# hjsuh94/irs_mpc

Hardware: NVIDIA B200
Metric: smoothed_dynamics_samples_per_s (higher is better)
Workload: dtype f32

## Files before the change

include/irs_mpc_b200.h:

```cpp
#ifndef IRS_MPC_B200_H
#define IRS_MPC_B200_H

#ifdef __cplusplus
extern "C" {
#endif

#define IRS_ABI_VERSION 3

enum { IRS_PENDULUM = 0, IRS_BICYCLE = 1, IRS_QUADROTOR = 2, IRS_THREE_CART = 3, IRS_MLP_2_1 = 4 };

int irs_mlp_register(int dim_x, int dim_u, int h1, int h2, const float* W1, const float* b1, const float* W2,
                     const float* b2, const float* W3, const float* b3, int* handle);
int irs_mlp_release(int handle);

enum {
  IRS_SAMPLES_BATCH_VARIANT = 1,
  IRS_PROJECT_ABSOLUTE = 2,
  IRS_PROJECT_DELTA = 4,
  IRS_ANTITHETIC = 8,
  IRS_CENTERED = 16
};

int irs_abi_version(void);
const char* irs_last_error(void);

int irs_set_gram_engine(int engine);

int irs_system_dims(int system, int* n, int* m, int* nj);

int irs_partial_width(int system, int order);

int irs_smooth_plan(int system, int order, int P, long long N, long long chunk_samples, int* C, long long* S);

int irs_smooth_zero_order_accumulate(int system, const double* params_host, int nparams, int flags,
                                     const double* x_nom, const double* u_nom, int P, long long N,
                                     const float* sigma_host, const float* noise,
                                     unsigned long long seed, unsigned iter, unsigned stream_id,
                                     unsigned p0, unsigned long long i0,
                                     int C, long long S, float* partials, void* stream);

int irs_smooth_first_order_accumulate(int system, const double* params_host, int nparams, int flags,
                                      const double* x_nom, const double* u_nom, int P, long long N,
                                      const float* sigma_host, const float* noise,
                                      unsigned long long seed, unsigned iter, unsigned stream_id,
                                      unsigned p0, unsigned long long i0,
                                      int C, long long S, float* partials, void* stream);

int irs_smooth_reduce_chunks(int system, int order, const float* partials, int P, int C,
                             double* reduced, void* stream);

int irs_smooth_finalize(int system, const double* params_host, int nparams, int order,
                        const double* x_nom, const double* u_nom, int P, int C,
                        const float* partials, const double* reduced, int nranks,
                        long long rank_stride, double n_total, int centered,
                        double* At, double* Bt, double* ct, int* status, void* stream);

int irs_smooth_finalize_peer(int system, const double* params_host, int nparams, int order,
                             const double* x_nom, const double* u_nom, int P, int C, const float* partials,
                             const void* peer_bufs_dev, const void* peer_flags_dev, int* epoch_dev,
                             unsigned int* done_counter, long long slot_stride, int flag_stride,
                             int rank, int world, double timeout_s, double n_total, int centered, int prepushed,
                             double* At, double* Bt, double* ct, int* status, void* stream);
int irs_smooth_finalize_peer_capacity(int system, int order, int* max_points);

int irs_smooth_push_supported(int system, int order);
int irs_smooth_zero_order_accumulate_push(int system, const double* params_host, int nparams, int flags,
                                          const double* x_nom, const double* u_nom, int P, long long N,
                                          const float* sigma_host, const float* noise,
                                          unsigned long long seed, unsigned iter, unsigned stream_id,
                                          unsigned p0, unsigned long long i0,
                                          int C, long long S, float* partials,
                                          const void* peer_bufs_dev, const void* peer_flags_dev, const int* epoch_dev,
                                          unsigned int* point_counters, long long slot_stride, int flag_stride,
                                          int rank, int world, void* stream);

int irs_smooth_finalize_gather(int system, const double* params_host, int nparams, int order,
                               const double* x_nom, const double* u_nom, int P, int C, const float* partials,
                               const void* peer_out_bufs_dev, const void* peer_flags_dev, int* epoch_dev,
                               unsigned int* done_counter, long long out_stride, int p0, int P_total,
                               int rank, int world, double timeout_s, double n_total, int centered,
                               double* ct_scratch, void* stream);

int irs_exact_linearize(int system, const double* params_host, int nparams,
                        const double* x_nom, const double* u_nom, int P,
                        double* At, double* Bt, double* ct, void* stream);

int irs_philox_dump(int P, long long N, int d, const float* sigma_host, unsigned long long seed,
                    unsigned iter, unsigned stream_id, unsigned p0, unsigned long long i0, int antithetic,
// ... 83 lines not shown
```

irs_mpc_b200/_lib.py:

```python
import ctypes
import os
import subprocess

_HERE = os.path.dirname(os.path.abspath(__file__))
LIB_PATH = os.environ.get("IRS_MPC_B200_LIB") or os.path.join(_HERE, "libirs_mpc_b200.so")
CSRC = os.path.join(_HERE, "csrc")
INCLUDE = os.path.join(os.path.dirname(_HERE), "include")

ABI_VERSION = 3

NVCC_FLAGS = ["-gencode", "arch=compute_100a,code=sm_100a", "-O3", "-lineinfo", "-std=c++17",
              "-shared", "-Xcompiler", "-fPIC"]


def sources():
    return [os.path.join(CSRC, "api.cu")]


def _stale():
    if not os.path.exists(LIB_PATH):
        return True
    t = os.path.getmtime(LIB_PATH)
    deps = [os.path.join(CSRC, f) for f in os.listdir(CSRC)] + [os.path.join(INCLUDE, "irs_mpc_b200.h")]
    return any(os.path.getmtime(d) > t for d in deps)
# ... 10 lines not shown
    return LIB_PATH


_c_double_p = ctypes.POINTER(ctypes.c_double)
_vp = ctypes.c_void_p
_ll = ctypes.c_longlong
_ull = ctypes.c_ulonglong
_i = ctypes.c_int
_u = ctypes.c_uint

SIGNATURES = {
    "irs_abi_version": [],
    "irs_last_error": [],
    "irs_set_gram_engine": [_i],
    "irs_system_dims": [_i, ctypes.POINTER(_i), ctypes.POINTER(_i), ctypes.POINTER(_i)],
    "irs_partial_width": [_i, _i],
    "irs_smooth_plan": [_i, _i, _i, _ll, _ll, ctypes.POINTER(_i), ctypes.POINTER(_ll)],
    "irs_smooth_zero_order_accumulate": [_i, _c_double_p, _i, _i, _vp, _vp, _i, _ll, _vp, _vp,
                                         _ull, _u, _u, _u, _ull, _i, _ll, _vp, _vp],
    "irs_smooth_first_order_accumulate": [_i, _c_double_p, _i, _i, _vp, _vp, _i, _ll, _vp, _vp,
                                          _ull, _u, _u, _u, _ull, _i, _ll, _vp, _vp],
    "irs_smooth_reduce_chunks": [_i, _i, _vp, _i, _i, _vp, _vp],
    "irs_smooth_finalize_peer": [_i, _c_double_p, _i, _i, _vp, _vp, _i, _i, _vp, _vp, _vp, _vp, _vp, _ll, _i,
                                 _i, _i, ctypes.c_double, ctypes.c_double, _i, _i, _vp, _vp, _vp, _vp, _vp],
    "irs_smooth_push_supported": [_i, _i],
    "irs_smooth_zero_order_accumulate_push": [_i, _c_double_p, _i, _i, _vp, _vp, _i, _ll, _vp, _vp,
                                              _ull, _u, _u, _u, _ull, _i, _ll, _vp,
                                              _vp, _vp, _vp, _vp, _ll, _i, _i, _i, _vp],
    "irs_smooth_finalize_peer_capacity": [_i, _i, ctypes.POINTER(_i)],
    "irs_smooth_finalize_gather": [_i, _c_double_p, _i, _i, _vp, _vp, _i, _i, _vp, _vp, _vp, _vp, _vp, _ll, _i, _i,
                                   _i, _i, ctypes.c_double, ctypes.c_double, _i, _vp, _vp],
    "irs_smooth_finalize": [_i, _c_double_p, _i, _i, _vp, _vp, _i, _i, _vp, _vp, _i, _ll,
                            ctypes.c_double, _i, _vp, _vp, _vp, _vp, _vp],
    "irs_exact_linearize": [_i, _c_double_p, _i, _vp, _vp, _i, _vp, _vp, _vp, _vp],
    "irs_philox_dump": [_i, _ll, _i, _vp, _ull, _u, _u, _u, _ull, _i, _vp, _vp, _vp],
    "irs_dynamics_batch_f32": [_i, _c_double_p, _i, _i, _vp, _vp, _vp, _ll, _vp],
    "irs_dynamics_batch_f64": [_i, _c_double_p, _i, _i, _vp, _vp, _vp, _ll, _vp],
    "irs_jacobian_xu_batch_f32": [_i, _c_double_p, _i, _vp, _vp, _vp, _ll, _vp],
    "irs_jacobian_xu_batch_f64": [_i, _c_double_p, _i, _vp, _vp, _vp, _ll, _vp],
    "irs_project_batch_f64": [_i, _c_double_p, _i, _vp, _ll, _vp],
    "irs_tvlqr_riccati": [_i, _i, _vp, _vp, _vp, _vp, _vp, _vp, _vp, _ll, _i, _i, _vp, _vp, _vp, _vp],
    "irs_tvlqr_riccati_segment": [_i, _i, _vp, _vp, _vp, _vp, _vp, _vp, _vp, _ll, _i, _i, _i, _i, _vp, _vp, _vp, _vp, _vp],
    "irs_tvlqr_riccati_ex": [_i, _i, _vp, _vp, _vp, _vp, _vp, _vp, _vp, _ll, _i, _i, _vp, _vp, _vp, _vp, _vp, _vp],
    "irs_mlp_register": [_i, _i, _i, _i, _vp, _vp, _vp, _vp, _vp, _vp, _vp],
    "irs_mlp_release": [_i],
    "irs_cem_refit": [_vp, _vp, _i, _i, _i, _i, _vp, _vp, _vp, _vp],
    "irs_gram_block_f64": [_i, _i, _vp, _vp, _ll, _vp, _vp],
    "irs_tvlqr_plan_rows": [_i, _i, _vp, _vp, _vp, _vp, _vp, _i, _i, _vp, _vp],
    "irs_tvlqr_plan_check": [_i, _i, _vp, _vp, _vp, _vp, _vp, _vp, _vp, _vp, _vp, _vp, ctypes.c_double, _i, _i, _i,
                             _vp, _vp, _vp],
    "irs_tvlqr_box_solve": [_i, _c_double_p, _i, _i, _vp, _vp, _vp, _vp, _vp, _vp, _vp, _vp, _vp, _vp, _ll, _vp, _vp,
                            _vp, _vp, _vp, _vp, _ll, _ll, _vp, _vp, _vp, ctypes.c_double, ctypes.c_double, ctypes.c_double,
                            _i, _i, _i, _vp, _vp, _vp, _vp, _vp, _vp],
    "irs_tvlqr_linear_rollout": [_i, _i, _vp, _vp, _vp, _vp, _vp, _vp, _i, _i, _vp, _vp, _vp],
    "irs_rollout_closed_loop": [_i, _c_double_p, _i, _vp, _vp, _vp, _vp, _ll, _vp, _vp, _i, _i,
                                _vp, _vp, _vp, _vp],
    "irs_rollout_open_loop": [_i, _c_double_p, _i, _vp, _vp, _vp, _ll, _vp, _vp, _i, _i,
                              _vp, _vp, _vp],
    "irs_fp32_fma_peak": [_i, _vp, _ll, _c_double_p, _vp],
    "irs_evaluate_cost": [_i, _i, _vp, _vp, _vp, _ll, _vp, _vp, _i, _i, _vp, _vp],
    "irs_graph_begin": [_vp],
    "irs_graph_end": [_vp, ctypes.POINTER(_vp)],
    "irs_graph_update_smoothing": [_vp, _vp, _ull, _u, _u],
    "irs_graph_launch": [_vp, _vp],
    "irs_graph_destroy": [_vp],
}
# ... 39 lines not shown
```

irs_mpc_b200/csrc/api.cu:

```cuda
#include <cstdarg>
#include <cstdio>
#include <cstdlib>
#include <cstring>
#include <mutex>
#include <vector>

#include "../../include/irs_mpc_b200.h"
#include "smooth.cuh"
#include "smooth_tc.cuh"
#include "tvlqr.cuh"
#include "tvlqr_box.cuh"
#include "cem.cuh"
#include "smooth_mlp.cuh"

namespace irs {

static thread_local char g_error[512] = "";

void set_error(const char* fmt, ...) {
    va_list ap;
    va_start(ap, fmt);
    vsnprintf(g_error, sizeof(g_error), fmt, ap);
    va_end(ap);
}
// ... 542 lines not shown

static const FinalizeTables* finalize_tables(int system) {
    const FinalizeTables* base = nullptr;
    if (cudaGetSymbolAddress((void**)&base, g_finalize_tables) != cudaSuccess) return nullptr;
    return base + system;
}

static int finalize_resident_blocks(int system, int order, int* out) {
    int per_sm = 0;
    cudaError_t e = cudaSuccess;
    if (order == 0) {
        IRS_DISPATCH_SYSTEM(system, double, Sys,
                            (e = cudaOccupancyMaxActiveBlocksPerMultiprocessor(
                                 &per_sm, finalize_zero_order_kernel<Sys, kFinalizeThreads>, kFinalizeThreads, 0)));
    } else {
        switch (system) {
            case kPendulum: e = cudaOccupancyMaxActiveBlocksPerMultiprocessor(&per_sm, finalize_first_order_kernel<Pendulum<double>>, kFinalizeThreads, 0); break;
            case kBicycle: e = cudaOccupancyMaxActiveBlocksPerMultiprocessor(&per_sm, finalize_first_order_kernel<Bicycle<double>>, kFinalizeThreads, 0); break;
            case kQuadrotor: e = cudaOccupancyMaxActiveBlocksPerMultiprocessor(&per_sm, finalize_first_order_kernel<Quadrotor<double>>, kFinalizeThreads, 0); break;
            case kMlp21: e = cudaOccupancyMaxActiveBlocksPerMultiprocessor(&per_sm, finalize_first_order_kernel<Mlp21<double>>, kFinalizeThreads, 0); break;
            default: set_error("system %d has no first-order path", system); return 1;
        }
    }
    if (e != cudaSuccess) return check_launch("cudaOccupancyMaxActiveBlocksPerMultiprocessor");
    *out = per_sm * num_sms();
    return 0;
}

static int smooth_finalize_impl(int system, const double* params_host, int nparams, int order,
                                const double* x_nom, const double* u_nom, int P, int C,
                                const float* partials, const double* reduced, int nranks,
                                long long rank_stride, double n_total, int centered,
                                double* At, double* Bt, double* ct, int* status, const PeerFusedArgs* peer,
                                void* stream) {
    FinalizeArgs a;
    if (load_params(system, params_host, nparams, &a.prm)) return 1;
    IRS_REQUIRE(order == 0 || order == 1, "order must be 0 or 1");
    IRS_REQUIRE(x_nom && u_nom && At && Bt && ct && status, "null pointer argument");
    IRS_REQUIRE((partials != nullptr) != (reduced != nullptr),
                "exactly one of partials (fp32 per-chunk) and reduced (fp64) must be given");
    a.reduced = reduced;
    IRS_REQUIRE(P >= 1 && C >= 1 && nranks >= 1 && n_total >= 1.0, "bad finalize arguments");
    IRS_REQUIRE(!(order == 1 && system == kThreeCart), "three_cart has no Jacobian");
    IRS_REQUIRE(!centered || (system == kThreeCart && order == 0), "centred accumulation is built for three_cart only");
    a.centered = centered ? 1 : 0;
    a.x_nom = x_nom;  a.u_nom = u_nom;  a.partials = partials;  a.rank_stride = rank_stride;
    a.R = nranks;  a.P = P;  a.C = C;  a.n_total = n_total;
    a.At = At;  a.Bt = Bt;  a.ct = ct;  a.status = status;
    memset(&a.peer, 0, sizeof(a.peer));
    if (peer != nullptr) a.peer = *peer;
    cudaStream_t st = (cudaStream_t)stream;
    a.tables = finalize_tables(system);
    if (a.tables == nullptr) return check_launch("finalize index tables") ? 1 : (set_error("finalize index tables"), 1);
    bool quad = P > 8 * num_sms();
    if (const char* e = getenv("IRS_FINALIZE_VARIANT")) {
        if (!strcmp(e, "block")) quad = false;
        else if (!strcmp(e, "quad")) quad = true;
    }
    if (peer != nullptr) quad = false;
    if (centered) quad = false;
    if (quad || order == 1) {
        IRS_DISPATCH_SYSTEM(system, double, Sys,
                            (dyn_batch_kernel<double, Sys><<<grid_for(P, 128), 128, 0, st>>>(a.prm, 0, x_nom, u_nom, ct, P)));
        if (check_launch("nominal dynamics kernel")) return 1;
    }
    const unsigned grid = (unsigned)P;
    if (order == 0) {
        if (quad) {
            IRS_DISPATCH_SYSTEM(system, double, Sys, {
                using QC = FinalizeQuadCfg<Sys>;
                auto kern = finalize_zero_order_quad_kernel<Sys>;
                if (cudaFuncSetAttribute(kern, cudaFuncAttributeMaxDynamicSharedMemorySize, (int)QC::kSmemBytes) != cudaSuccess)
                    return check_launch("cudaFuncSetAttribute(finalize_zero_order_quad_kernel)");
                kern<<<(unsigned)((P + QC::PPB - 1) / QC::PPB), kFinalizeQuadThreads, QC::kSmemBytes, st>>>(a);
            });
        } else {
            IRS_DISPATCH_SYSTEM(system, double, Sys,
                                (finalize_zero_order_kernel<Sys, kFinalizeThreads><<<grid, kFinalizeThreads, 0, st>>>(a)));
        }
    } else {
        switch (system) {
            case kPendulum: finalize_first_order_kernel<Pendulum<double>><<<grid, kFinalizeThreads, 0, st>>>(a); break;
            case kBicycle: finalize_first_order_kernel<Bicycle<double>><<<grid, kFinalizeThreads, 0, st>>>(a); break;
            case kQuadrotor: finalize_first_order_kernel<Quadrotor<double>><<<grid, kFinalizeThreads, 0, st>>>(a); break;
            case kMlp21: finalize_first_order_kernel<Mlp21<double>><<<grid, kFinalizeThreads, 0, st>>>(a); break;
            default: set_error("unknown system id %d", system); return 1;
        }
    }
    return check_launch("finalize_kernel");
}

int irs_smooth_finalize(int system, const double* params_host, int nparams, int order,
                        const double* x_nom, const double* u_nom, int P, int C,
                        const float* partials, const double* reduced, int nranks,
                        long long rank_stride, double n_total, int centered,
                        double* At, double* Bt, double* ct, int* status, void* stream) {
    return smooth_finalize_impl(system, params_host, nparams, order, x_nom, u_nom, P, C, partials, reduced, nranks,
                                rank_stride, n_total, centered, At, Bt, ct, status, nullptr, stream);
}

int irs_smooth_finalize_peer_capacity(int system, int order, int* max_points) {
    IRS_REQUIRE(system >= 0 && system < kNumSystems && (order == 0 || order == 1) && max_points, "bad arguments");
    return finalize_resident_blocks(system, order, max_points);
}

int irs_smooth_finalize_peer(int system, const double* params_host, int nparams, int order,
                             const double* x_nom, const double* u_nom, int P, int C, const float* partials,
                             const void* peer_bufs_dev, const void* peer_flags_dev, int* epoch_dev,
                             unsigned int* done_counter, long long slot_stride, int flag_stride,
                             int rank, int world, double timeout_s, double n_total, int centered, int prepushed,
                             double* At, double* Bt, double* ct, int* status, void* stream) {
    IRS_REQUIRE(system >= 0 && system < kNumSystems, "unknown system id %d", system);
    IRS_REQUIRE(partials && peer_bufs_dev && peer_flags_dev && epoch_dev && done_counter, "null pointer argument");
    IRS_REQUIRE(world >= 1 && world <= kFinalizeThreads && rank >= 0 && rank < world, "bad rank / world");
    IRS_REQUIRE(timeout_s > 0.0, "timeout must be positive");
    const int width = irs_partial_width(system, order);
    IRS_REQUIRE(slot_stride >= (long long)P * width && flag_stride >= P, "exchange buffers too small for P=%d", P);
    int resident = 0;
    if (finalize_resident_blocks(system, order, &resident)) return 1;
    IRS_REQUIRE(P <= resident, "the fused exchange needs its %d blocks co-resident (%d fit): use the all-gather path", P, resident);
    PeerFusedArgs px{(double* const*)peer_bufs_dev, (int* const*)peer_flags_dev, epoch_dev, done_counter,
                     slot_stride, flag_stride, rank, world, (unsigned long long)(timeout_s * 1e9),
                     kPeerExchange, 0, 0, 0, prepushed ? 1 : 0};
    return smooth_finalize_impl(system, params_host, nparams, order, x_nom, u_nom, P, C, partials, nullptr, 1, 0,
                                n_total, centered, At, Bt, ct, status, &px, stream);
}

int irs_smooth_finalize_gather(int system, const double* params_host, int nparams, int order,
                               const double* x_nom, const double* u_nom, int P, int C, const float* partials,
                               const void* peer_out_bufs_dev, const void* peer_flags_dev, int* epoch_dev,
                               unsigned int* done_counter, long long out_stride, int p0, int P_total,
                               int rank, int world, double timeout_s, double n_total, int centered,
                               double* ct_scratch, void* stream) {
    IRS_REQUIRE(system >= 0 && system < kNumSystems, "unknown system id %d", system);
    IRS_REQUIRE(peer_out_bufs_dev && peer_flags_dev && epoch_dev && done_counter, "null pointer argument");
    IRS_REQUIRE(world >= 1 && world <= kFinalizeThreads && rank >= 0 && rank < world, "bad rank / world");
    IRS_REQUIRE(timeout_s > 0.0 && P >= 0 && p0 >= 0 && P_total >= 1 && p0 + P <= P_total, "bad gather arguments");
    const SystemDims dm = system_dims(system);
    IRS_REQUIRE(out_stride >= (long long)P_total * (dm.n * (dm.n + dm.m + 1) + 1), "output buffers too small");
    PeerFusedArgs px{(double* const*)peer_out_bufs_dev, (int* const*)peer_flags_dev, epoch_dev, done_counter,
                     0, 0, rank, world, (unsigned long long)(timeout_s * 1e9), kPeerGather, p0, P_total, out_stride, 0};
    if (P == 0) {
        peer_gather_wait_kernel<<<1, 128, 0, (cudaStream_t)stream>>>(px);
        return check_launch("peer_gather_wait_kernel");
    }
    IRS_REQUIRE(partials && ct_scratch, "null pointer argument");
    return smooth_finalize_impl(system, params_host, nparams, order, x_nom, u_nom, P, C, partials, nullptr, 1, 0,
                                n_total, centered, ct_scratch, ct_scratch, ct_scratch, (int*)ct_scratch, &px, stream);
}

int irs_exact_linearize(int system, const double* params_host, int nparams,
                        const double* x_nom, const double* u_nom, int P,
                        double* At, double* Bt, double* ct, void* stream) {
    SysParams prm;
    if (load_params(system, params_host, nparams, &prm)) return 1;
    IRS_REQUIRE(system != kThreeCart,
                "three_cart is not differentiable and has no Jacobian (three_cart_dynamics.py:20)");
    IRS_REQUIRE(x_nom && u_nom && At && Bt && ct, "null pointer argument");
    IRS_REQUIRE(P >= 1, "need at least one nominal point");
    cudaStream_t st = (cudaStream_t)stream;
    switch (system) {
        case kPendulum: exact_linearize_kernel<Pendulum<double>><<<(P + 63) / 64, 64, 0, st>>>(prm, x_nom, u_nom, P, At, Bt, ct); break;
        case kBicycle: exact_linearize_kernel<Bicycle<double>><<<(P + 63) / 64, 64, 0, st>>>(prm, x_nom, u_nom, P, At, Bt, ct); break;
        case kQuadrotor: exact_linearize_kernel<Quadrotor<double>><<<(P + 63) / 64, 64, 0, st>>>(prm, x_nom, u_nom, P, At, Bt, ct); break;
        case kMlp21: exact_linearize_kernel<Mlp21<double>><<<(P + 63) / 64, 64, 0, st>>>(prm, x_nom, u_nom, P, At, Bt, ct); break;
        default: set_error("unknown system id %d", system); return 1;
    }
    return check_launch("exact_linearize_kernel");
}

int irs_mlp_register(int dim_x, int dim_u, int h1, int h2, const float* W1, const float* b1, const float* W2,
                     const float* b2, const float* W3, const float* b3, int* handle) {
    IRS_REQUIRE(W1 && b1 && W2 && b2 && W3 && b3 && handle, "null pointer argument");
    IRS_REQUIRE(dim_x >= 1 && dim_u >= 1, "need dim_x >= 1 and dim_u >= 1");
    IRS_REQUIRE(h1 >= 1 && h1 <= kMlpMaxHidden && h2 >= 1 && h2 <= kMlpMaxHidden,
                "hidden widths must lie in [1, %d], got %d and %d", kMlpMaxHidden, h1, h2);
    const int d = dim_x + dim_u, n = dim_x;
    const long long count = MlpView::floats(d, n, h1, h2);
    std::vector<float> host((size_t)count);
    MlpView v(host.data(), d, n, h1, h2);
    memcpy(const_cast<float*>(v.w1), W1, sizeof(float) * h1 * d);
// ... 440 lines not shown
```

irs_mpc_b200/csrc/common.cuh:

```cuda
#pragma once
#include <cuda_runtime.h>
#include <stdint.h>

namespace irs {

void set_error(const char* fmt, ...);
int check_launch(const char* what);

#define IRS_REQUIRE(cond, ...)            \
    do {                                  \
        if (!(cond)) {                    \
            irs::set_error(__VA_ARGS__);  \
            return 1;                     \
        }                                 \
    } while (0)

struct SysParams {
    double v[10];
    float f[20];
    const float* mlp;
    const unsigned short* mlp_w2;
    int h1, h2;
};

template <typename R>
struct Math;

template <>
struct Math<float> {
    static __device__ __forceinline__ void sincos(float a, float& s, float& c) {
        __sincosf(a, &s, &c);
    }
    static __device__ __forceinline__ float rcp(float a) {
        float r;
        asm("rcp.approx.ftz.f32 %0, %1;" : "=f"(r) : "f"(a));
        return r;
    }
    static __device__ __forceinline__ float div(float a, float b) { return __fdividef(a, b); }
};

template <>
struct Math<double> {
    static __device__ __forceinline__ void sincos(double a, double& s, double& c) {
        ::sincos(a, &s, &c);
    }
    static __device__ __forceinline__ double rcp(double a) { return 1.0 / a; }
    static __device__ __forceinline__ double div(double a, double b) { return a / b; }
};

constexpr int kPhiloxRounds = 7;
constexpr uint32_t kPhiloxM0 = 0xD2511F53u;
constexpr uint32_t kPhiloxM1 = 0xCD9E8D57u;
constexpr uint32_t kPhiloxW0 = 0x9E3779B9u;
constexpr uint32_t kPhiloxW1 = 0xBB67AE85u;

template <int ROUNDS = kPhiloxRounds>
// ... 61 lines not shown
```

irs_mpc_b200/csrc/smooth.cuh:

```cuda
#pragma once
#include "systems.cuh"

namespace irs {

enum SmoothFlags {
    kFlagSamplesBatchVariant = 1,
    kFlagProjectAbsolute = 2,
    kFlagProjectDelta = 4,
    kFlagAntithetic = 8,
    kFlagCentered = 16,
};

struct PeerPushArgs {
    double* const* peer_bufs;
    int* const* peer_flags;
    const int* epoch;
    unsigned int* counters;
    long long slot_stride;
    int flag_stride;
    int rank, world;
};

struct SmoothArgs {
    const double* x_nom;
// ... 356 lines not shown
    const int c = blockIdx.x % a.C;
    const long long s_begin = (long long)c * a.S;
    const long long s_end = s_begin + a.S < a.N ? s_begin + a.S : a.N;
    float xbar[n], ubar[m], fbar[n];
#pragma unroll
    for (int q = 0; q < n; ++q) xbar[q] = (float)a.x_nom[(long long)p * n + q];
#pragma unroll
    for (int q = 0; q < m; ++q) ubar[q] = (float)a.u_nom[(long long)p * m + q];
#pragma unroll
    for (int q = 0; q < n; ++q) fbar[q] = 0.f;
    float acc[NJ];
#pragma unroll
    for (int k = 0; k < NJ; ++k) acc[k] = 0.f;
    for (long long s = s_begin + threadIdx.x; s < s_end; s += 128) {
        float w[RS];
        make_sample<Sys, false, RS>(sys, a, p, s, xbar, ubar, fbar, w, false);
        float v[NJ];
        sys.jac_var(w, w + n, v);
#pragma unroll
        for (int k = 0; k < NJ; ++k) acc[k] += v[k];
    }
    const int lane = threadIdx.x & 31, warp = threadIdx.x >> 5;
#pragma unroll
    for (int k = 0; k < NJ; ++k) {
        const float s = warp_sum(acc[k]);
        if (lane == 0) slab[warp][k] = s;
    }
    __syncthreads();
    float* out = a.partials + ((long long)p * a.C + c) * NJ;
    for (int k = threadIdx.x; k < NJ; k += 128) out[k] = (slab[0][k] + slab[1][k]) + (slab[2][k] + slab[3][k]);
}

constexpr int kFinalizeThreads = 128;

constexpr int kMaxGramEntries = kMaxRegressors * (kMaxRegressors + 1) / 2 + kMaxRegressors * kMaxRegressors;
constexpr int kMaxTriEntries = kMaxRegressors * (kMaxRegressors + 1) / 2;
struct FinalizeTables {
    unsigned char gram_i[kMaxGramEntries], gram_j[kMaxGramEntries];
    unsigned char tri_r[kMaxTriEntries], tri_c[kMaxTriEntries];
};
constexpr FinalizeTables make_finalize_tables(int n, int m) {
    FinalizeTables t{};
    const int d = n + m, W = d + n;
    int e = 0;
    for (int i = 0; i < d; ++i)
        for (int j = i; j < W; ++j, ++e) { t.gram_i[e] = (unsigned char)i;  t.gram_j[e] = (unsigned char)j; }
    e = 0;
    for (int r = 0; r < d; ++r)
        for (int c = 0; c <= r; ++c, ++e) { t.tri_r[e] = (unsigned char)r;  t.tri_c[e] = (unsigned char)c; }
    return t;
}
__device__ const FinalizeTables g_finalize_tables[kNumSystems] = {
    make_finalize_tables(2, 1), make_finalize_tables(5, 2), make_finalize_tables(12, 4), make_finalize_tables(6, 2),
    make_finalize_tables(2, 1)};

struct PeerFusedArgs {
    double* const* peer_bufs;
    int* const* peer_flags;
    int* epoch;
    unsigned int* done_counter;
    long long slot_stride;
    int flag_stride;
    int rank, world;
    unsigned long long timeout_ns;
    int mode;
    int p0, P_total;
    long long out_stride;
    int prepushed;
};
enum PeerMode { kPeerNone = 0, kPeerExchange = 1, kPeerGather = 2 };

struct FinalizeArgs {
    const double* x_nom;
    const double* u_nom;
    const float* partials;
    const double* reduced;
    long long rank_stride;
    int R;
    int P, C;
    double n_total;
    double* At;
    double* Bt;
    double* ct;
    int* status;
    const FinalizeTables* tables;
    int centered;
    PeerFusedArgs peer;
    SysParams prm;
};

struct PartialSource {
    const float* partials;
    const double* reduced;
    long long rank_stride;
    int R, C;
};
__device__ __forceinline__ PartialSource partial_source(const FinalizeArgs& a) {
    return PartialSource{a.partials, a.reduced, a.rank_stride, a.R, a.C};
}

__device__ __forceinline__ double sum_partials(const PartialSource& a, int p, int e, int width) {
    double s = 0.0;
    if (a.reduced != nullptr) {
        const double* src = a.reduced + (long long)p * width + e;
        int r = 0;
        for (; r + 8 <= a.R; r += 8) {
            double v[8];
#pragma unroll
            for (int k = 0; k < 8; ++k) v[k] = __ldcg(src + (long long)(r + k) * a.rank_stride);
#pragma unroll
            for (int k = 0; k < 8; ++k) s += v[k];
        }
        if (r + 4 <= a.R) {
            double v[4];
#pragma unroll
            for (int k = 0; k < 4; ++k) v[k] = __ldcg(src + (long long)(r + k) * a.rank_stride);
#pragma unroll
            for (int k = 0; k < 4; ++k) s += v[k];
            r += 4;
// ... 260 lines not shown
    for (int q = 0; q < n; ++q) nom[n + m + q] = fb[q];
}

template <class Sys, int BT>
__device__ __forceinline__ void write_abc(const FinalizeArgs& a, int p, const double* AB,
                                          const double* nom , int tid) {
    constexpr int n = Sys::N, m = Sys::M, d = Sys::D;
    for (int e = tid; e < n * d; e += BT) {
        const int r = e / d, cidx = e % d;
        if (cidx < n) a.At[((long long)p * n + r) * n + cidx] = AB[e];
        else a.Bt[((long long)p * n + r) * m + (cidx - n)] = AB[e];
    }
    if (tid < n) {
        double acc = nom[d + tid];
#pragma unroll
        for (int q = 0; q < d; ++q) acc = fma(-AB[tid * d + q], nom[q], acc);
        a.ct[(long long)p * n + tid] = acc;
    }
}

template <class Sys, int BT>
__global__ void __launch_bounds__(BT, 1) finalize_zero_order_kernel(const FinalizeArgs a) {
    constexpr int n = Sys::N, m = Sys::M, d = Sys::D;
    constexpr int NACC = gram_nacc(n, m);
    constexpr int WIDTH = gram_width_of<Sys>();
    __shared__ double Gm[d * d];
    __shared__ double Bm[d * n];
    __shared__ double sAB[n * d];
    __shared__ double inv_diag[d];
    __shared__ double nom[d + n];
    __shared__ double mom[WIDTH - NACC > 0 ? WIDTH - NACC : 1];
    __shared__ double spread[d];
    __shared__ double rho[n];
    const int tid = threadIdx.x, lane = tid & 31;
    const int p = blockIdx.x;
    PartialSource src = partial_source(a);
    bool peer_late = false;
    int epoch = 0;
    if (a.peer.mode == kPeerExchange) epoch = peer_exchange_point<BT>(a, p, WIDTH, tid, &src, &peer_late);
    else if (a.peer.mode == kPeerGather) epoch = *reinterpret_cast<volatile int*>(a.peer.epoch) + 1;
    __shared__ int status_s;
    {
        constexpr int NE = (WIDTH + BT - 1) / BT;
        int rel[NE];
#pragma unroll
        for (int q = 0; q < NE; ++q) rel[q] = tid + q * BT < WIDTH ? tid + q * BT : -1;
        double sums[NE];
        const long long pbase = (long long)p * (src.reduced != nullptr ? (long long)WIDTH : (long long)src.C * WIDTH);
        sum_partials_multi<NE>(src, pbase, rel, WIDTH, sums);
#pragma unroll
        for (int q = 0; q < NE; ++q) {
            if (rel[q] >= NACC) {
                mom[rel[q] - NACC] = sums[q];
            } else if (rel[q] >= 0) {
                const int i = a.tables->gram_i[rel[q]], j = a.tables->gram_j[rel[q]];
                if (j < d) {
                    Gm[i * d + j] = sums[q];
                    Gm[j * d + i] = sums[q];
                } else {
                    Bm[i * n + (j - d)] = sums[q];
                }
            }
        }
    }
    if constexpr (WIDTH > NACC) {
        if (a.centered && tid == 32) {
            const Sys sys(a.prm);
            double xb[n], ub[m], x2[n], u2[m], f2[n], fb[n];
#pragma unroll
            for (int q = 0; q < n; ++q) { xb[q] = a.x_nom[(long long)p * n + q];  x2[q] = 2.0 * xb[q]; }
#pragma unroll
            for (int q = 0; q < m; ++q) { ub[q] = a.u_nom[(long long)p * m + q];  u2[q] = 2.0 * ub[q]; }
            sys.template step<true>(x2, u2, f2);
            sys.template step<false>(xb, ub, fb);
#pragma unroll
            for (int q = 0; q < n; ++q) rho[q] = f2[q] - fb[q];
        }
    }
    __syncthreads();
    if (tid < d) spread[tid] = Gm[tid * d + tid];
    if constexpr (WIDTH > NACC) {
        if (a.centered) {
            __syncthreads();
            for (int e = tid; e < d * d; e += BT) {
                const int i = e / d, j = e % d;
                const double si = i < n ? a.x_nom[(long long)p * n + i] : a.u_nom[(long long)p * m + (i - n)];
                const double sj = j < n ? a.x_nom[(long long)p * n + j] : a.u_nom[(long long)p * m + (j - n)];
                Gm[e] = fma(a.n_total * si, sj, fma(si, mom[j], fma(mom[i], sj, Gm[e])));
            }
            for (int e = tid; e < d * n; e += BT) {
                const int i = e / n, q = e % n;
                const double si = i < n ? a.x_nom[(long long)p * n + i] : a.u_nom[(long long)p * m + (i - n)];
                Bm[e] = fma(a.n_total * si, rho[q], fma(si, mom[d + q], fma(mom[i], rho[q], Bm[e])));
            }
        }
    }
    __syncthreads();
    constexpr bool kWarpNominal = is_mlp<Sys>::value;
    __shared__ float mlp_act[kWarpNominal ? 2 * kMlpMaxHidden : 1];
    if (kWarpNominal ? (tid >= 32 && tid < 64) : (tid == 32)) {
        if constexpr (kWarpNominal) {
            const Sys sys(a.prm);
            double xb[n], ub[m], fb[n];
#pragma unroll
            for (int q = 0; q < n; ++q) xb[q] = a.x_nom[(long long)p * n + q];
#pragma unroll
            for (int q = 0; q < m; ++q) ub[q] = a.u_nom[(long long)p * m + q];
            sys.step_warp(xb, ub, fb, mlp_act, mlp_act + kMlpMaxHidden, tid - 32);
            if (tid == 32) {
#pragma unroll
                for (int q = 0; q < n; ++q) nom[q] = xb[q];
#pragma unroll
                for (int q = 0; q < m; ++q) nom[n + q] = ub[q];
#pragma unroll
                for (int q = 0; q < n; ++q) nom[n + m + q] = fb[q];
            }
        } else {
            nominal_compute_to_smem<Sys>(a, p, nom);
        }
    } else if (tid < 32) {
        bool bad = false;
        double row[d];
#pragma unroll
        for (int j = 0; j < d; ++j) row[j] = (lane < d && j <= lane) ? Gm[lane * d + j] : 0.0;
        static_for<0, d>([&](auto kc) {
            constexpr int k = decltype(kc)::value;
            double lk[k > 0 ? k : 1];
            static_for<0, k>([&](auto jc) { constexpr int j = decltype(jc)::value;  lk[j] = __shfl_sync(0xffffffffu, row[j], k); });
            const double d0 = __shfl_sync(0xffffffffu, row[k], k);
            double dk = d0;
            static_for<0, k>([&](auto jc) { constexpr int j = decltype(jc)::value;  dk = fma(-lk[j], lk[j], dk); });
            bool zero_col = false;
            const double scale_k = (WIDTH > NACC && a.centered) ? spread[k] : d0;
            if (d0 == 0.0) { zero_col = true; dk = 1.0; }
            else if (!(dk > 1e-6 * scale_k)) { bad = true; dk = 1.0; }
            const double ikk = rsqrt(dk);
            double sk = row[k];
            static_for<0, k>([&](auto jc) { constexpr int j = decltype(jc)::value;  sk = fma(-row[j], lk[j], sk); });
            if (lane > k) row[k] = zero_col ? 0.0 : sk * ikk;
            if (lane == k) { row[k] = dk * ikk;  inv_diag[k] = ikk; }
            if (zero_col)
                for (int q = lane; q < n; q += 32) Bm[k * n + q] = 0.0;
        });
        if (lane < d) {
#pragma unroll
            for (int j = 0; j < d; ++j)
                if (j <= lane) Gm[lane * d + j] = row[j];
        }
        __syncwarp();
        if (lane < n) {
            const int q = lane;
            double y[d];
// ... 314 lines not shown
```

irs_mpc_b200/csrc/smooth_tc.cuh:

```cuda
#pragma once
#include "smooth.cuh"

#ifndef IRS_TC_NOM_BATCH
#define IRS_TC_NOM_BATCH 64
#endif
#ifndef IRS_TC_PACK_TMEM
#define IRS_TC_PACK_TMEM 1
#endif
#ifndef IRS_TC_MIN_BLOCKS
#define IRS_TC_MIN_BLOCKS 4
#endif

namespace irs {

__device__ __forceinline__ uint32_t smem_u32(const void* p) {
    return (uint32_t)__cvta_generic_to_shared(p);
}

__device__ __forceinline__ uint64_t umma_smem_desc(uint32_t saddr, uint32_t lbo_bytes, uint32_t sbo_bytes) {
    uint64_t d = 0;
    d |= (uint64_t)((saddr & 0x3FFFF) >> 4);
    d |= (uint64_t)((lbo_bytes >> 4) & 0x3FFF) << 16;
    d |= (uint64_t)((sbo_bytes >> 4) & 0x3FFF) << 32;
    d |= (uint64_t)1 << 46;
// ... 98 lines not shown
    __shared__ double nom64_s[n + m];
    __shared__ float scratch[C::kRows * kScr];
    __shared__ uint16_t idx_s[C::NACC];
    __shared__ float mom_s[C::kWarps][kMom];
    __shared__ int push_flag_s;

    const int tid = threadIdx.x, lane = tid & 31;
    const int warp = __shfl_sync(0xffffffffu, tid >> 5, 0);
    const long long num_items = (long long)a.P * a.C;

    if (tid == 0) {
#pragma unroll
        for (int w = 0; w < C::kWarps; ++w) {
#pragma unroll
            for (int s = 0; s < NSTAGE; ++s) mbar_init(&mbar_empty[w][s], 1);
            mbar_init(&mbar_done[w], 1);
        }
        asm volatile("fence.mbarrier_init.release.cluster;");
    }
    for (int e = tid; e < C::NACC; e += C::kThreads) {
        int i = 0;
        while (i + 1 < d && gram_row_offset(i + 1, C::W) <= e) ++i;
        idx_s[e] = (uint16_t)((i << 8) | (i + (e - gram_row_offset(i, C::W))));
    }
    if constexpr (DUAL) {
        for (int e = tid; e < NSTAGE * C::kWarps * C::kStageBytes / 16; e += C::kThreads)
            reinterpret_cast<uint4*>(stage_mem)[e] = make_uint4(0u, 0u, 0u, 0u);
    }
    if (warp == 0) {
        asm volatile("tcgen05.alloc.cta_group::1.sync.aligned.shared::cta.b32 [%0], %1;" ::"r"(smem_u32(&tmem_base_s)),
                     "r"(C::kTmemCols));
        asm volatile("tcgen05.relinquish_alloc_permit.cta_group::1.sync.aligned;");
    }
    const Sys sys(a.prm);
    auto nominal_point = [&](int p, int slot, float (&xb)[n], float (&ub)[m], float (&fb)[n]) {
        double xd[n], ud[m];
#pragma unroll
        for (int q = 0; q < n; ++q) {
            xd[q] = a.x_nom[(long long)p * n + q];
            if (q < 4) pos64_tab[slot][q] = xd[q];
        }
#pragma unroll
        for (int q = 0; q < m; ++q) ud[q] = a.u_nom[(long long)p * m + q];
        if constexpr (CENTERED) {
            centred_frame<Sys>(xd, ud, xb, ub);
            if (a.flags & kFlagSamplesBatchVariant) sys.template step<true>(xb, ub, fb);
            else sys.template step<false>(xb, ub, fb);
        } else {
#pragma unroll
            for (int q = 0; q < n; ++q) xb[q] = (float)xd[q];
#pragma unroll
            for (int q = 0; q < m; ++q) ub[q] = (float)ud[q];
            sys.template step<false>(xb, ub, fb);
        }
    };
    auto prepare_nominals = [&](long long first) {
        if (tid < kNomBatch) {
            const long long it2 = first + (long long)tid * gridDim.x;
            if (it2 < num_items) {
                float xb[n], ub[m], fb[n];
                nominal_point((int)(it2 / a.C), tid, xb, ub, fb);
                float* row = nom_tab[tid];
#pragma unroll
                for (int q = 0; q < n; ++q) row[q] = xb[q];
#pragma unroll
                for (int q = 0; q < m; ++q) row[n + q] = ub[q];
// ... 355 lines not shown
```

irs_mpc_b200/smoothing.py:

```python
import ctypes

import numpy as np
import torch

from . import _device, _lib

ZERO_ORDER = 0
FIRST_ORDER = 1
FLAG_PROJECT_ABSOLUTE, FLAG_PROJECT_DELTA, FLAG_ANTITHETIC, FLAG_CENTERED = 2, 4, 8, 16


def plan(system_id, order, P, N, chunk_samples=0):
    C = ctypes.c_int(0)
    S = ctypes.c_longlong(0)
    _lib.call("irs_smooth_plan", system_id, order, P, N, int(chunk_samples), ctypes.byref(C), ctypes.byref(S))
    return C.value, S.value


class Workspace:

    def __init__(self, system, order, P, N, chunk_samples=0):
        self.key = (system.system_id, order, P, N) if not chunk_samples else (system.system_id, order, P, N, chunk_samples)
        self.C, self.S = plan(system.system_id, order, P, N, chunk_samples)
        self.width = _lib.lib().irs_partial_width(system.system_id, order)
        n, m = system.dim_x, system.dim_u
        self.P, self.n, self.m = P, n, m
        self.partials = _device.empty((P, self.C, self.width), torch.float32)
        na, nb, nc = P * n * n, P * n * m, P * n
        self._out = _device.empty((na + nb + nc + (P + 1) // 2,))
        self.At = self._out[:na].view(P, n, n)
        self.Bt = self._out[na:na + nb].view(P, n, m)
        self.ct = self._out[na + nb:na + nb + nc].view(P, n)
        self.status = self._out[na + nb + nc:].view(torch.int32)[:P]
        self._nom = _device.empty((P * (n + m),))
        self.x_nom = self._nom[:P * n].view(P, n)
        self.u_nom = self._nom[P * n:].view(P, m)
        self._out_host = None
        self._nom_host = None
        self.centered = False

    def _host_buffers(self):
        if self._nom_host is None:
            self._nom_host = torch.empty(self._nom.shape, dtype=torch.float64).pin_memory()
            self._out_host = torch.empty(self._out.shape, dtype=torch.float64).pin_memory()
            self._nom_host_np = self._nom_host.numpy()
            self._out_host_np = self._out_host.numpy()

    def stage_nominal(self, x_trj, u_trj):
        P, n, m = self.P, self.n, self.m
        self._host_buffers()
        h = self._nom_host_np
        h[:P * n] = np.asarray(x_trj, dtype=np.float64)[:P].reshape(-1)
        h[P * n:] = np.asarray(u_trj, dtype=np.float64)[:P].reshape(-1)

    def enqueue_upload(self):
        self._host_buffers()
        self._nom.copy_(self._nom_host, non_blocking=True)

    def enqueue_download(self):
        self._host_buffers()
        self._out_host.copy_(self._out, non_blocking=True)

    def read_download(self):
        P, n, m = self.P, self.n, self.m
        torch.cuda.current_stream().synchronize()
        h = self._out_host_np.copy()
        na, nb, nc = P * n * n, P * n * m, P * n
        At = h[:na].reshape(P, n, n)
        Bt = h[na:na + nb].reshape(P, n, m)
        ct = h[na + nb:na + nb + nc].reshape(P, n)
        status = h[na + nb + nc:].view(np.int32)[:P]
        return At, Bt, ct, status

    def h2d_bytes(self):
        return self._nom.numel() * 8

    def d2h_bytes(self):
        return self._out.numel() * 8


def accumulate(system, order, x_nom, u_nom, N, ws, sigma=None, noise=None, seed=0, it=1,
               stream_id=0, p0=0, i0=0, flags=0, point_range=None):
    partials = ws.partials
    if point_range is not None:
        lo, hi = point_range
        x_nom, u_nom, partials = x_nom[lo:hi], u_nom[lo:hi], partials[lo:hi]
        noise = None if noise is None else noise[lo:hi]
        p0 += lo
    P = x_nom.shape[0]
    prm, nprm = system._params()
    if system.batch_differs_from_scalar and order == ZERO_ORDER:
        flags |= 1
    ws.centered = order == ZERO_ORDER and bool(flags & (FLAG_PROJECT_ABSOLUTE | FLAG_CENTERED))
    sig = None
    if noise is None:
        sig = np.ascontiguousarray(np.asarray(sigma, dtype=np.float32))
        if sig.shape != (system.dim_x + system.dim_u,):
            raise ValueError("sigma must have n + m = %d entries" % (system.dim_x + system.dim_u))
        sig = sig.ctypes.data_as(ctypes.c_void_p)
    fn = ("irs_smooth_zero_order_accumulate" if order == ZERO_ORDER
          else "irs_smooth_first_order_accumulate")
    _lib.call(fn, system.system_id, prm, nprm, flags, _device.ptr(x_nom), _device.ptr(u_nom), P,
              int(N), sig, _device.ptr(noise), int(seed), int(it), int(stream_id),
              int(p0), int(i0), ws.C, ws.S, _device.ptr(partials), _device.stream_ptr())


def reduce_chunks(system, order, ws, out=None):
    P = ws.partials.shape[0]
    if out is None:
        out = _device.empty((P, ws.width))
    _lib.call("irs_smooth_reduce_chunks", system.system_id, order, _device.ptr(ws.partials), P, ws.C,
              _device.ptr(out), _device.stream_ptr())
    return out


def finalize(system, order, x_nom, u_nom, ws, n_total, partials=None, reduced=None, nranks=1,
             rank_stride=0, point_range=None):
    prm, nprm = system._params()
    part = None if reduced is not None else (ws.partials if partials is None else partials)
    At, Bt, ct, status = ws.At, ws.Bt, ws.ct, ws.status
    if point_range is not None:
        lo, hi = point_range
        assert reduced is None and nranks == 1
        x_nom, u_nom, part = x_nom[lo:hi], u_nom[lo:hi], part[lo:hi]
        At, Bt, ct, status = At[lo:hi], Bt[lo:hi], ct[lo:hi], status[lo:hi]
    P = x_nom.shape[0]
    _lib.call("irs_smooth_finalize", system.system_id, prm, nprm, order, _device.ptr(x_nom),
              _device.ptr(u_nom), P, ws.C, _device.ptr(part), _device.ptr(reduced), nranks,
              int(rank_stride), float(n_total), 1 if ws.centered else 0, _device.ptr(At), _device.ptr(Bt),
              _device.ptr(ct), _device.ptr(status), _device.stream_ptr())
    return ws.At, ws.Bt, ws.ct, ws.status


def linearize(system, order, x_nom, u_nom, N, ws=None, **kw):
    P = x_nom.shape[0]
    if ws is None or ws.key != (system.system_id, order, P, N):
        ws = Workspace(system, order, P, N)
    accumulate(system, order, x_nom, u_nom, N, ws, **kw)
    return finalize(system, order, x_nom, u_nom, ws, N) + (ws,)


def check_status(status):
    if isinstance(status, torch.Tensor):
        status = status.detach().cpu().numpy()
    status = np.asarray(status)
    if not status.any():
        return
    late = int(np.count_nonzero(status == 2))
    if late:
        raise RuntimeError(
            "peer exchange timed out: the Gram blocks of %d nominal point(s) did not arrive from every rank "
            "(a rank is missing, far behind, or issued a different call sequence); the fit was NOT computed"
            % late)
    bad = int(np.count_nonzero(status))
    raise np.linalg.LinAlgError(
        "smoothing fit: the sample Gram matrix [dx du]^T[dx du] is rank deficient at %d "
        "nominal point(s) (too few samples, NaN in the dynamics, or regressors whose offset dwarfs "
        "their spread — three_cart's projection='absolute' quirk far from the origin: the Gram is "
        "accumulated in fp32)" % bad)
```

Baseline: 69.26 billion.

## Overlap zero-order finalize with accumulate via PDL and stage partials through cp.async

```diff
diff --git a/include/irs_mpc_b200.h b/include/irs_mpc_b200.h
--- a/include/irs_mpc_b200.h
+++ b/include/irs_mpc_b200.h
@@ -54,6 +54,12 @@
                         const float* partials, const double* reduced, int nranks,
                         long long rank_stride, double n_total, int centered,
                         double* At, double* Bt, double* ct, int* status, void* stream);
+
+int irs_smooth_finalize_ex(int system, const double* params_host, int nparams, int order,
+                           const double* x_nom, const double* u_nom, int P, int C,
+                           const float* partials, const double* reduced, int nranks,
+                           long long rank_stride, double n_total, int centered,
+                           double* At, double* Bt, double* ct, int* status, int follows_accumulate, void* stream);
 
 int irs_smooth_finalize_peer(int system, const double* params_host, int nparams, int order,
                              const double* x_nom, const double* u_nom, int P, int C, const float* partials,
diff --git a/irs_mpc_b200/_lib.py b/irs_mpc_b200/_lib.py
--- a/irs_mpc_b200/_lib.py
+++ b/irs_mpc_b200/_lib.py
@@ -66,6 +66,8 @@
                                    _i, _i, ctypes.c_double, ctypes.c_double, _i, _vp, _vp],
     "irs_smooth_finalize": [_i, _c_double_p, _i, _i, _vp, _vp, _i, _i, _vp, _vp, _i, _ll,
                             ctypes.c_double, _i, _vp, _vp, _vp, _vp, _vp],
+    "irs_smooth_finalize_ex": [_i, _c_double_p, _i, _i, _vp, _vp, _i, _i, _vp, _vp, _i, _ll,
+                               ctypes.c_double, _i, _vp, _vp, _vp, _vp, _i, _vp],
     "irs_exact_linearize": [_i, _c_double_p, _i, _vp, _vp, _i, _vp, _vp, _vp, _vp],
     "irs_philox_dump": [_i, _ll, _i, _vp, _ull, _u, _u, _u, _ull, _i, _vp, _vp, _vp],
     "irs_dynamics_batch_f32": [_i, _c_double_p, _i, _i, _vp, _vp, _vp, _ll, _vp],
diff --git a/irs_mpc_b200/csrc/api.cu b/irs_mpc_b200/csrc/api.cu
--- a/irs_mpc_b200/csrc/api.cu
+++ b/irs_mpc_b200/csrc/api.cu
@@ -598,7 +598,7 @@
                                 const float* partials, const double* reduced, int nranks,
                                 long long rank_stride, double n_total, int centered,
                                 double* At, double* Bt, double* ct, int* status, const PeerFusedArgs* peer,
-                                void* stream) {
+                                int follows_accumulate, void* stream) {
     FinalizeArgs a;
     if (load_params(system, params_host, nparams, &a.prm)) return 1;
     IRS_REQUIRE(order == 0 || order == 1, "order must be 0 or 1");
@@ -610,6 +610,7 @@
     IRS_REQUIRE(!(order == 1 && system == kThreeCart), "three_cart has no Jacobian");
     IRS_REQUIRE(!centered || (system == kThreeCart && order == 0), "centred accumulation is built for three_cart only");
     a.centered = centered ? 1 : 0;
+    a.dependent = 0;
     a.x_nom = x_nom;  a.u_nom = u_nom;  a.partials = partials;  a.rank_stride = rank_stride;
     a.R = nranks;  a.P = P;  a.C = C;  a.n_total = n_total;
     a.At = At;  a.Bt = Bt;  a.ct = ct;  a.status = status;
@@ -641,8 +642,24 @@
                 kern<<<(unsigned)((P + QC::PPB - 1) / QC::PPB), kFinalizeQuadThreads, QC::kSmemBytes, st>>>(a);
             });
         } else {
-            IRS_DISPATCH_SYSTEM(system, double, Sys,
-                                (finalize_zero_order_kernel<Sys, kFinalizeThreads><<<grid, kFinalizeThreads, 0, st>>>(a)));
+            bool dependent = follows_accumulate && peer == nullptr && reduced == nullptr;
+            if (const char* e = getenv("IRS_FIT_PDL"))
+                if (atoi(e) == 0) dependent = false;
+            a.dependent = dependent ? 1 : 0;
+            cudaLaunchAttribute attr[1];
+            attr[0].id = cudaLaunchAttributeProgrammaticStreamSerialization;
+            attr[0].val.programmaticStreamSerializationAllowed = 1;
+            cudaLaunchConfig_t cfg = {};
+            cfg.gridDim = dim3(grid);
+            cfg.blockDim = dim3(kFinalizeThreads);
+            cfg.dynamicSmemBytes = 0;
+            cfg.stream = st;
+            cfg.attrs = attr;
+            cfg.numAttrs = dependent ? 1 : 0;
+            IRS_DISPATCH_SYSTEM(system, double, Sys, {
+                if (cudaLaunchKernelEx(&cfg, finalize_zero_order_kernel<Sys, kFinalizeThreads>, a) != cudaSuccess)
+                    return check_launch("finalize_zero_order_kernel");
+            });
         }
     } else {
         switch (system) {
@@ -662,7 +679,16 @@
                         long long rank_stride, double n_total, int centered,
                         double* At, double* Bt, double* ct, int* status, void* stream) {
     return smooth_finalize_impl(system, params_host, nparams, order, x_nom, u_nom, P, C, partials, reduced, nranks,
-                                rank_stride, n_total, centered, At, Bt, ct, status, nullptr, stream);
+                                rank_stride, n_total, centered, At, Bt, ct, status, nullptr, 0, stream);
+}
+
+int irs_smooth_finalize_ex(int system, const double* params_host, int nparams, int order,
+                           const double* x_nom, const double* u_nom, int P, int C,
+                           const float* partials, const double* reduced, int nranks,
+                           long long rank_stride, double n_total, int centered,
+                           double* At, double* Bt, double* ct, int* status, int follows_accumulate, void* stream) {
+    return smooth_finalize_impl(system, params_host, nparams, order, x_nom, u_nom, P, C, partials, reduced, nranks,
+                                rank_stride, n_total, centered, At, Bt, ct, status, nullptr, follows_accumulate, stream);
 }
 
 int irs_smooth_finalize_peer_capacity(int system, int order, int* max_points) {
@@ -689,7 +715,7 @@
                      slot_stride, flag_stride, rank, world, (unsigned long long)(timeout_s * 1e9),
                      kPeerExchange, 0, 0, 0, prepushed ? 1 : 0};
     return smooth_finalize_impl(system, params_host, nparams, order, x_nom, u_nom, P, C, partials, nullptr, 1, 0,
-                                n_total, centered, At, Bt, ct, status, &px, stream);
+                                n_total, centered, At, Bt, ct, status, &px, 0, stream);
 }
 
 int irs_smooth_finalize_gather(int system, const double* params_host, int nparams, int order,
@@ -712,7 +738,7 @@
     }
     IRS_REQUIRE(partials && ct_scratch, "null pointer argument");
     return smooth_finalize_impl(system, params_host, nparams, order, x_nom, u_nom, P, C, partials, nullptr, 1, 0,
-                                n_total, centered, ct_scratch, ct_scratch, ct_scratch, (int*)ct_scratch, &px, stream);
+                                n_total, centered, ct_scratch, ct_scratch, ct_scratch, (int*)ct_scratch, &px, 0, stream);
 }
 
 int irs_exact_linearize(int system, const double* params_host, int nparams,
diff --git a/irs_mpc_b200/csrc/common.cuh b/irs_mpc_b200/csrc/common.cuh
--- a/irs_mpc_b200/csrc/common.cuh
+++ b/irs_mpc_b200/csrc/common.cuh
@@ -22,6 +22,9 @@
     const unsigned short* mlp_w2;
     int h1, h2;
 };
+
+__device__ __forceinline__ void griddep_launch_dependents() { asm volatile("griddepcontrol.launch_dependents;" ::: "memory"); }
+__device__ __forceinline__ void griddep_wait() { asm volatile("griddepcontrol.wait;" ::: "memory"); }
 
 template <typename R>
 struct Math;
diff --git a/irs_mpc_b200/csrc/smooth.cuh b/irs_mpc_b200/csrc/smooth.cuh
--- a/irs_mpc_b200/csrc/smooth.cuh
+++ b/irs_mpc_b200/csrc/smooth.cuh
@@ -412,6 +412,16 @@
 }
 
 constexpr int kFinalizeThreads = 128;
+template <int WIDTH>
+__host__ __device__ constexpr int finalize_stage_floats() {
+    return (10240 / WIDTH < 32 ? 10240 / WIDTH : 32) * WIDTH;
+}
+
+__device__ __forceinline__ void cp_async_f32(float* dst, const float* src) {
+    asm volatile("cp.async.ca.shared.global [%0], [%1], 4;" ::"r"((unsigned)__cvta_generic_to_shared(dst)), "l"(src)
+                 : "memory");
+}
+__device__ __forceinline__ void cp_async_wait_all() { asm volatile("cp.async.wait_all;" ::: "memory"); }
 
 constexpr int kMaxGramEntries = kMaxRegressors * (kMaxRegressors + 1) / 2 + kMaxRegressors * kMaxRegressors;
 constexpr int kMaxTriEntries = kMaxRegressors * (kMaxRegressors + 1) / 2;
@@ -465,6 +475,7 @@
     int* status;
     const FinalizeTables* tables;
     int centered;
+    int dependent;
     PeerFusedArgs peer;
     SysParams prm;
 };
@@ -791,8 +802,62 @@
     __shared__ double mom[WIDTH - NACC > 0 ? WIDTH - NACC : 1];
     __shared__ double spread[d];
     __shared__ double rho[n];
+    constexpr int kStage = finalize_stage_floats<WIDTH>();
+    __shared__ float stage[kStage];
     const int tid = threadIdx.x, lane = tid & 31;
     const int p = blockIdx.x;
+    constexpr bool kWarpNominal = is_mlp<Sys>::value;
+    __shared__ float mlp_act[kWarpNominal ? 2 * kMlpMaxHidden : 1];
+    const bool nominal_thread = kWarpNominal ? (tid >= 32 && tid < 64) : (tid == 32);
+    auto response_shift = [&]() {
+        if constexpr (WIDTH > NACC) {
+            const Sys sys(a.prm);
+            double xb[n], ub[m], x2[n], u2[m], f2[n], fb[n];
+#pragma unroll
+            for (int q = 0; q < n; ++q) { xb[q] = a.x_nom[(long long)p * n + q];  x2[q] = 2.0 * xb[q]; }
+#pragma unroll
+            for (int q = 0; q < m; ++q) { ub[q] = a.u_nom[(long long)p * m + q];  u2[q] = 2.0 * ub[q]; }
+            sys.template step<true>(x2, u2, f2);
+            sys.template step<false>(xb, ub, fb);
+#pragma unroll
+            for (int q = 0; q < n; ++q) rho[q] = f2[q] - fb[q];
+        }
+    };
+    auto nominal_response = [&]() {
+        if constexpr (kWarpNominal) {
+            const Sys sys(a.prm);
+            double xb[n], ub[m], fb[n];
+#pragma unroll
+            for (int q = 0; q < n; ++q) xb[q] = a.x_nom[(long long)p * n + q];
+#pragma unroll
+            for (int q = 0; q < m; ++q) ub[q] = a.u_nom[(long long)p * m + q];
+            sys.step_warp(xb, ub, fb, mlp_act, mlp_act + kMlpMaxHidden, tid - 32);
+            if (tid == 32) {
+#pragma unroll
+                for (int q = 0; q < n; ++q) nom[q] = xb[q];
+#pragma unroll
+                for (int q = 0; q < m; ++q) nom[n + q] = ub[q];
+#pragma unroll
+                for (int q = 0; q < n; ++q) nom[n + m + q] = fb[q];
+            }
+        } else {
+            nominal_compute_to_smem<Sys>(a, p, nom);
+        }
+    };
+    constexpr int NE = (WIDTH + BT - 1) / BT;
+    int rel[NE], gi[NE], gj[NE];
+#pragma unroll
+    for (int q = 0; q < NE; ++q) {
+        rel[q] = tid + q * BT < WIDTH ? tid + q * BT : -1;
+        const bool g = rel[q] >= 0 && rel[q] < NACC;
+        gi[q] = g ? a.tables->gram_i[rel[q]] : 0;
+        gj[q] = g ? a.tables->gram_j[rel[q]] : 0;
+    }
+    if (a.dependent && nominal_thread) {
+        if (WIDTH > NACC && a.centered) response_shift();
+        nominal_response();
+    }
+    griddep_wait();
     PartialSource src = partial_source(a);
     bool peer_late = false;
     int epoch = 0;
@@ -800,19 +865,33 @@
     else if (a.peer.mode == kPeerGather) epoch = *reinterpret_cast<volatile int*>(a.peer.epoch) + 1;
     __shared__ int status_s;
     {
-        constexpr int NE = (WIDTH + BT - 1) / BT;
-        int rel[NE];
-#pragma unroll
-        for (int q = 0; q < NE; ++q) rel[q] = tid + q * BT < WIDTH ? tid + q * BT : -1;
         double sums[NE];
         const long long pbase = (long long)p * (src.reduced != nullptr ? (long long)WIDTH : (long long)src.C * WIDTH);
-        sum_partials_multi<NE>(src, pbase, rel, WIDTH, sums);
+        const int rows = src.R * src.C;
+        if (src.reduced == nullptr && rows * WIDTH <= kStage) {
+            const int cw = src.C * WIDTH;
+            for (int r = 0; r < src.R; ++r) {
+                const float* g = src.partials + r * src.rank_stride + pbase;
+                for (int i = tid; i < cw; i += BT) cp_async_f32(&stage[r * cw + i], g + i);
+            }
+            cp_async_wait_all();
+            __syncthreads();
+#pragma unroll
+            for (int q = 0; q < NE; ++q) {
+                double s = 0.0;
+                if (rel[q] >= 0)
+                    for (int row = 0; row < rows; ++row) s += (double)stage[row * WIDTH + rel[q]];
+                sums[q] = s;
+            }
+        } else {
+            sum_partials_multi<NE>(src, pbase, rel, WIDTH, sums);
+        }
 #pragma unroll
         for (int q = 0; q < NE; ++q) {
             if (rel[q] >= NACC) {
                 mom[rel[q] - NACC] = sums[q];
             } else if (rel[q] >= 0) {
-                const int i = a.tables->gram_i[rel[q]], j = a.tables->gram_j[rel[q]];
+                const int i = gi[q], j = gj[q];
                 if (j < d) {
                     Gm[i * d + j] = sums[q];
                     Gm[j * d + i] = sums[q];
@@ -822,20 +901,7 @@
             }
         }
     }
-    if constexpr (WIDTH > NACC) {
-        if (a.centered && tid == 32) {
-            const Sys sys(a.prm);
-            double xb[n], ub[m], x2[n], u2[m], f2[n], fb[n];
-#pragma unroll
-            for (int q = 0; q < n; ++q) { xb[q] = a.x_nom[(long long)p * n + q];  x2[q] = 2.0 * xb[q]; }
-#pragma unroll
-            for (int q = 0; q < m; ++q) { ub[q] = a.u_nom[(long long)p * m + q];  u2[q] = 2.0 * ub[q]; }
-            sys.template step<true>(x2, u2, f2);
-            sys.template step<false>(xb, ub, fb);
-#pragma unroll
-            for (int q = 0; q < n; ++q) rho[q] = f2[q] - fb[q];
-        }
-    }
+    if (WIDTH > NACC && !a.dependent && a.centered && tid == 32) response_shift();
     __syncthreads();
     if (tid < d) spread[tid] = Gm[tid * d + tid];
     if constexpr (WIDTH > NACC) {
@@ -855,28 +921,8 @@
         }
     }
     __syncthreads();
-    constexpr bool kWarpNominal = is_mlp<Sys>::value;
-    __shared__ float mlp_act[kWarpNominal ? 2 * kMlpMaxHidden : 1];
-    if (kWarpNominal ? (tid >= 32 && tid < 64) : (tid == 32)) {
-        if constexpr (kWarpNominal) {
-            const Sys sys(a.prm);
-            double xb[n], ub[m], fb[n];
-#pragma unroll
-            for (int q = 0; q < n; ++q) xb[q] = a.x_nom[(long long)p * n + q];
-#pragma unroll
-            for (int q = 0; q < m; ++q) ub[q] = a.u_nom[(long long)p * m + q];
-            sys.step_warp(xb, ub, fb, mlp_act, mlp_act + kMlpMaxHidden, tid - 32);
-            if (tid == 32) {
-#pragma unroll
-                for (int q = 0; q < n; ++q) nom[q] = xb[q];
-#pragma unroll
-                for (int q = 0; q < m; ++q) nom[n + q] = ub[q];
-#pragma unroll
-                for (int q = 0; q < n; ++q) nom[n + m + q] = fb[q];
-            }
-        } else {
-            nominal_compute_to_smem<Sys>(a, p, nom);
-        }
+    if (nominal_thread) {
+        if (!a.dependent) nominal_response();
     } else if (tid < 32) {
         bool bad = false;
         double row[d];
diff --git a/irs_mpc_b200/csrc/smooth_tc.cuh b/irs_mpc_b200/csrc/smooth_tc.cuh
--- a/irs_mpc_b200/csrc/smooth_tc.cuh
+++ b/irs_mpc_b200/csrc/smooth_tc.cuh
@@ -154,6 +154,7 @@
                      "r"(C::kTmemCols));
         asm volatile("tcgen05.relinquish_alloc_permit.cta_group::1.sync.aligned;");
     }
+    griddep_launch_dependents();
     const Sys sys(a.prm);
     auto nominal_point = [&](int p, int slot, float (&xb)[n], float (&ub)[m], float (&fb)[n]) {
         double xd[n], ud[m];
diff --git a/irs_mpc_b200/smoothing.py b/irs_mpc_b200/smoothing.py
--- a/irs_mpc_b200/smoothing.py
+++ b/irs_mpc_b200/smoothing.py
@@ -38,6 +38,7 @@
         self._out_host = None
         self._nom_host = None
         self.centered = False
+        self.accumulated_on = None
 
     def _host_buffers(self):
         if self._nom_host is None:
@@ -100,9 +101,11 @@
         sig = sig.ctypes.data_as(ctypes.c_void_p)
     fn = ("irs_smooth_zero_order_accumulate" if order == ZERO_ORDER
           else "irs_smooth_first_order_accumulate")
+    stream = _device.stream_ptr()
     _lib.call(fn, system.system_id, prm, nprm, flags, _device.ptr(x_nom), _device.ptr(u_nom), P,
               int(N), sig, _device.ptr(noise), int(seed), int(it), int(stream_id),
-              int(p0), int(i0), ws.C, ws.S, _device.ptr(partials), _device.stream_ptr())
+              int(p0), int(i0), ws.C, ws.S, _device.ptr(partials), stream)
+    ws.accumulated_on = stream
 
 
 def reduce_chunks(system, order, ws, out=None):
@@ -117,6 +120,9 @@
 def finalize(system, order, x_nom, u_nom, ws, n_total, partials=None, reduced=None, nranks=1,
              rank_stride=0, point_range=None):
     prm, nprm = system._params()
+    stream = _device.stream_ptr()
+    follows = ws.accumulated_on is not None and ws.accumulated_on == stream
+    ws.accumulated_on = None
     part = None if reduced is not None else (ws.partials if partials is None else partials)
     At, Bt, ct, status = ws.At, ws.Bt, ws.ct, ws.status
     if point_range is not None:
@@ -125,10 +131,10 @@
         x_nom, u_nom, part = x_nom[lo:hi], u_nom[lo:hi], part[lo:hi]
         At, Bt, ct, status = At[lo:hi], Bt[lo:hi], ct[lo:hi], status[lo:hi]
     P = x_nom.shape[0]
-    _lib.call("irs_smooth_finalize", system.system_id, prm, nprm, order, _device.ptr(x_nom),
+    _lib.call("irs_smooth_finalize_ex", system.system_id, prm, nprm, order, _device.ptr(x_nom),
               _device.ptr(u_nom), P, ws.C, _device.ptr(part), _device.ptr(reduced), nranks,
               int(rank_stride), float(n_total), 1 if ws.centered else 0, _device.ptr(At), _device.ptr(Bt),
-              _device.ptr(ct), _device.ptr(status), _device.stream_ptr())
+              _device.ptr(ct), _device.ptr(status), 1 if follows else 0, stream)
     return ws.At, ws.Bt, ws.ct, ws.status
 
 
```

After: 70.78 billion, median of 6. +2.2%, better.
